# Orange-OpenSource/AIVC

Hardware: AMD Instinct MI355X
Metric: encode+decode fps @1080p YUV420 (RA GOP32) (higher is better)
Workload: dtype f32; 1 GPU; 1920x1080 8-bit YUV420, coding structure 1_GOP_32: one 128-frame clip = 4 intra-period units of 33 frames (132 coded frames, the last 4 repeat the last frame) encoded + decoded per step; synthetic random-init stand-in for model ms_ssim-4 (widths {'n2': 64, 'n': 128, 'c_y': 64, 'c_short': 64, 'c_z': 32, 'n_h': 128}), last analysis conv calibrated so that 6 (MOFNet) / 12 (CodecNet) of the 64 y featu; parallelism=single GPU

## Files before the change

aivc_amd/csrc/common.h:

```cpp
#pragma once
#include <hip/hip_runtime.h>
#include <stdint.h>

#include <atomic>

#include "../../include/aivc_detmath.h"
#include "../../include/aivc_hip.h"

#define AIVC_EXPORT extern "C" __attribute__((visibility("default")))

namespace aivc {

void set_last_error(const char *msg);
int check_launch(const char *what);

struct LdsOptIn {
  std::atomic<uint64_t> done{0};
  bool raise(const void *fn, size_t bytes) {
    int dev = 0;
    if (hipGetDevice(&dev) != hipSuccess) return false;
    const uint64_t bit = 1ull << (dev & 63);
    if (done.load(std::memory_order_acquire) & bit) return true;
    if (hipFuncSetAttribute(fn, hipFuncAttributeMaxDynamicSharedMemorySize, (int)bytes) != hipSuccess) return false;
    done.fetch_or(bit, std::memory_order_release);
    return true;
  }
};

constexpr uint64_t LOADER_MAX_BYTES = 0xFFFFFFF0ull;
static inline bool loader_addressable(uint64_t bytes) { return bytes <= LOADER_MAX_BYTES; }

static inline hipStream_t to_stream(aivc_stream_t s) { return reinterpret_cast<hipStream_t>(s); }
static inline unsigned cdiv(size_t a, size_t b) { return (unsigned)((a + b - 1) / b); }

__device__ __forceinline__ float act_apply(int act, float v) {
  switch (act) {
    case AIVC_ACT_LEAKY: return v > 0.0f ? v : v * 0.01f;
    case AIVC_ACT_RELU: return v > 0.0f ? v : 0.0f;
    case AIVC_ACT_SIGMOID: return aivc_sigmoidf_det(v);
    default: return v;
  }
}

constexpr float GDN_SAFE_LO = 0x1p-60f, GDN_SAFE_HI = 0x1p60f;
__device__ __forceinline__ float sqrt_rn_safe(float s) {
  const float y = __builtin_amdgcn_rsqf(s);
  float g = s * y, h = 0.5f * y;
  const float e = __builtin_fmaf(-h, g, 0.5f);
  h = __builtin_fmaf(h, e, h);
  g = __builtin_fmaf(g, e, g);
  const float d = __builtin_fmaf(-g, g, s);
  return __builtin_fmaf(d, h, g);
}
__device__ __forceinline__ float div_rn_safe(float v, float d) {
  float r = __builtin_amdgcn_rcpf(d);
  const float e = __builtin_fmaf(-d, r, 1.0f);
  r = __builtin_fmaf(e, r, r);
  float q = v * r;
  float t = __builtin_fmaf(-d, q, v);
  q = __builtin_fmaf(t, r, q);
  t = __builtin_fmaf(-d, q, v);
  return __builtin_fmaf(t, r, q);
}
__device__ __forceinline__ void gdn_range(float &mx, float &mn, float a, float s) {
  mx = __builtin_fmaxf(__builtin_fmaxf(mx, __builtin_fabsf(a)), s);
  mn = __builtin_fminf(__builtin_fminf(mn, __builtin_fabsf(a)), s);
}
__device__ __forceinline__ void gdn_range_pair(float &mx, float &mn, float s0, float s1) {
  mx = __builtin_fmaxf(__builtin_fmaxf(mx, s0), s1);
  mn = __builtin_fminf(__builtin_fminf(mn, s0), s1);
}
__device__ __forceinline__ bool gdn_range_ok(float mx, float mn) {
  return __builtin_amdgcn_ballot_w64(mn >= GDN_SAFE_LO && mx <= GDN_SAFE_HI) == __builtin_amdgcn_ballot_w64(true);
}

struct Epilogue {
  const float *bias, *mul, *res, *xin;
  float *y;
  int act1, act2, mode;
  __device__ __forceinline__ void store(size_t opix, int co, int c_out, float acc) const {
    float v = acc;
    if (bias) v = v + bias[co];
    if (mode == AIVC_MODE_GDN || mode == AIVC_MODE_IGDN) {
      const float xc = xin[opix * c_out + co];
      const float nrm = __builtin_sqrtf(v);
      v = (mode == AIVC_MODE_IGDN) ? xc * nrm : xc / nrm;
    }
    finish(opix, co, c_out, v);
  }
  __device__ __forceinline__ void finish(size_t opix, int co, int c_out, float v) const {
    v = act_apply(act1, v);
    const size_t o = opix * c_out + co;
    if (mul) v = mul[o] * v;
    if (res) v = v + res[o];
    v = act_apply(act2, v);
    y[o] = v;
  }
};

int conv2d_direct(const aivc_conv_params &p, hipStream_t s);
int conv2d_mfma(const aivc_conv_params &p, hipStream_t s);
bool conv2d_mfma_addressable(const aivc_conv_params &p);
bool conv2d_mfma_supported(const aivc_conv_params &p);
bool conv2d_mfma_tail_supported(const aivc_conv_params &p);
int conv2d_mfma_variant(const aivc_conv_params &p);
bool conv2d_bf16x3_supported(const aivc_conv_params &p);
int conv2d_bf16x3(const aivc_conv_params &p, hipStream_t s);
int split_weights_bf16x3(const float *w, int c_out, int k_total, void *out, hipStream_t s);
int conv2d_bf16x3_tile(const aivc_conv_params &p);
bool conv2d_wino_supported(const aivc_conv_params &p);
int conv2d_wino(const aivc_conv_params &p, hipStream_t s);
int conv2d_wino_variant(const aivc_conv_params &p);
int winograd_weights(const float *w, int c_out, int c_in, float *u, hipStream_t s);
int winograd_weights_poly5(const float *w, int c_out, int c_in, float *u, hipStream_t s);
int winograd_weights_tconv5(const float *w, int c_out, int c_in, float *u, hipStream_t s);
bool gdn_resident_supported(const aivc_conv_params &p);
int gdn_resident(const aivc_conv_params &p, hipStream_t s);
bool conv_images_supported(const aivc_image_src *src, int n_img, const aivc_conv_params &p);
int conv_images(const aivc_image_src *src, int n_img, const aivc_conv_params &p, hipStream_t s);
bool conv2d_thin_supported(const aivc_conv_params &p);
int conv2d_thin(const aivc_conv_params &p, hipStream_t s);
int conv2d_thin_variant(const aivc_conv_params &p);

}
```

aivc_amd/csrc/gdn.hip:

```cpp
#include <stdlib.h>

#include "mfma_util.h"

namespace aivc {

struct GdnArgs {
  aivc_conv_params p;
  int M;
  int ntiles;
};

constexpr int GDN_BM = 64;

__device__ __forceinline__ int gdn_swz(int row) { return (row & 15) ^ ((row & 4) << 1); }

template <int C>
struct GdnCfg {
  static constexpr int NB = C / 32;
  static constexpr int PW = C == 64 ? 2 : 1;
  static constexpr int NW = NB * PW;
  static constexpr int TM = 2 / PW;
  static constexpr int ROWB = C * 4;
  static constexpr int STAGE = GDN_BM * ROWB;
  static constexpr int PIECES = STAGE / 1024;
  static constexpr int PPW = (PIECES + NW - 1) / NW;
  static constexpr int WGS = C == 192 ? 1 : 2;
};

template <int C, bool INV, bool RES>
__global__ __launch_bounds__(64 * GdnCfg<C>::NW, GdnCfg<C>::WGS) void gdn_resident_kernel(GdnArgs a) {
  using Cfg = GdnCfg<C>;
  constexpr int NB = Cfg::NB, PW = Cfg::PW, NW = Cfg::NW, TM = Cfg::TM, ROWB = Cfg::ROWB, STAGE = Cfg::STAGE, PIECES = Cfg::PIECES, PPW = Cfg::PPW;
  constexpr int NOCT = C / 8;
  extern __shared__ __attribute__((aligned(16))) char gsmem[];
  const uint32_t lds0 = (uint32_t)(uintptr_t)(__attribute__((address_space(3))) char *)gsmem;
  const aivc_conv_params &p = a.p;
  const int tid = threadIdx.x, lane = tid & 63;
  const int wave = __builtin_amdgcn_readfirstlane(tid >> 6);
  const int nb = wave % NB, pw = wave / NB;
  const int l31 = lane & 31, hh = lane >> 5;
  const int M = a.M;

  float4 gb[NOCT];
  {
    const float *g = p.w + (size_t)(32 * nb + l31) * C + 4 * hh;
#pragma unroll
    for (int o = 0; o < NOCT; ++o) gb[o] = *reinterpret_cast<const float4 *>(g + 8 * o);
  }
  const float cbeta = p.bias[32 * nb + l31];

  uint32_t d_voff[PPW];
#pragma unroll
  for (int k = 0; k < PPW; ++k) {
    const int q = wave + NW * k;
    const int b = q * 1024 + lane * 16;
    const int row = b / ROWB, chunk = ((b % ROWB) >> 4) ^ gdn_swz(row);
    d_voff[k] = (uint32_t)(row * ROWB + chunk * 16);
  }
  const uint32_t w_dst = __builtin_amdgcn_readfirstlane(lds0 + (uint32_t)wave * 1024u);
  auto issue = [&](int tile, int stage) {
    const int m0 = tile * GDN_BM;
    const float *src = p.x + (size_t)m0 * C;
    const uint32_t dst = w_dst + (uint32_t)(stage * STAGE);
    if (m0 + GDN_BM <= M) {
#pragma unroll
      for (int k = 0; k < PPW; ++k)
        if (PIECES % NW == 0 || wave + NW * k < PIECES) glds16(src, d_voff[k], dst + (uint32_t)(NW * k) * 1024u);
    } else {
      const int last = M - 1 - m0;
#pragma unroll
      for (int k = 0; k < PPW; ++k)
        if (PIECES % NW == 0 || wave + NW * k < PIECES)
          glds16(src, (uint32_t)min((int)(d_voff[k] / ROWB), last) * (uint32_t)ROWB + d_voff[k] % ROWB, dst + (uint32_t)(NW * k) * 1024u);
    }
  };

  const int frow = (PW == 2 ? 32 * pw : 0) + l31;
  int f_off[8];
#pragma unroll
  for (int o = 0; o < 8; ++o) f_off[o] = frow * ROWB + (((2 * o + hh) ^ gdn_swz(frow)) << 4);
  const int e_chunk = (8 * nb + (l31 >> 2)) ^ (hh ? 12 : 0);
  const int e_lane = 4 * hh * ROWB + (l31 & 3) * 4;
  const int rb0 = PW == 2 ? 32 * pw : 0;

  const int G = gridDim.x;
  int tile = blockIdx.x;
  if (tile >= a.ntiles) return;
  issue(tile, 0);
  int stage = 0;
  for (; tile < a.ntiles; tile += G, stage ^= 1) {
    asm volatile("s_waitcnt vmcnt(0)" ::: "memory");
    __builtin_amdgcn_s_barrier();
    if (tile + G < a.ntiles) issue(tile + G, stage ^ 1);
    const char *sb = gsmem + stage * STAGE;

    floatx16 acc[TM];
    typedef float f32x2 __attribute__((ext_vector_type(2)));
    struct Frag { f32x2 lo, hi; };
    Frag cur[TM], nxt[TM];
    auto read_frag = [&](Frag (&f)[TM], int o) {
#pragma unroll
      for (int i = 0; i < TM; ++i) {
        const float4 v = *reinterpret_cast<const float4 *>(sb + f_off[o & 7] + (o >> 3) * 256 + i * 32 * ROWB);
        f[i].lo = (f32x2){v.x, v.y};
        f[i].hi = (f32x2){v.z, v.w};
      }
    };
    read_frag(cur, 0);
#pragma unroll
    for (int o = 0; o < NOCT; ++o) {
      if (o + 1 < NOCT) read_frag(nxt, o + 1);
#pragma unroll
      for (int i = 0; i < TM; ++i) {
        cur[i].lo = cur[i].lo * cur[i].lo;
        cur[i].hi = cur[i].hi * cur[i].hi;
      }
      __builtin_amdgcn_sched_barrier(0);
#pragma unroll
      for (int s = 0; s < 4; ++s) {
        const float bv = s == 0 ? gb[o].x : (s == 1 ? gb[o].y : (s == 2 ? gb[o].z : gb[o].w));
#pragma unroll
        for (int i = 0; i < TM; ++i) {
          const float av = s == 0 ? cur[i].lo.x : (s == 1 ? cur[i].lo.y : (s == 2 ? cur[i].hi.x : cur[i].hi.y));
          if (o == 0 && s == 0) {
            const floatx16 zero = {0.0f, 0.0f, 0.0f, 0.0f, 0.0f, 0.0f, 0.0f, 0.0f, 0.0f, 0.0f, 0.0f, 0.0f, 0.0f, 0.0f, 0.0f, 0.0f};
            acc[i] = __builtin_amdgcn_mfma_f32_32x32x2f32(av, bv, zero, 0, 0, 0);
          } else {
            acc[i] = __builtin_amdgcn_mfma_f32_32x32x2f32(av, bv, acc[i], 0, 0, 0);
          }
        }
      }
      __builtin_amdgcn_sched_barrier(0);
#pragma unroll
      for (int i = 0; i < TM; ++i) cur[i] = nxt[i];
    }

    const int m0 = tile * GDN_BM;
    const int rows_left = M - m0;
    typedef __attribute__((address_space(1))) char gchar;
    typedef __attribute__((address_space(1))) float gfloat;
    typedef __attribute__((address_space(1))) const float cgfloat;
    gchar *yb = (gchar *)(uintptr_t)(p.y + (size_t)m0 * C);
    const gchar *rsb = (const gchar *)(uintptr_t)(p.res + (size_t)m0 * C);
    const uint32_t lane_b = (uint32_t)((4 * hh) * ROWB + (32 * nb + l31) * 4);
    auto epilogue = [&](auto WHOLE) {
      constexpr bool whole = decltype(WHOLE)::value;
      constexpr int EG = RES ? 4 : 8;
#pragma unroll
      for (int i = 0; i < TM; ++i)
#pragma unroll
      for (int r0 = 0; r0 < 16; r0 += EG) {
        const int rb = rb0 + 32 * i;
        float xv[EG], sv[EG], rv[EG];
        float mx = 1.0f, mn = 1.0f;
#pragma unroll
        for (int q = 0; q < EG; ++q) {
          const int r = r0 + q, rloc = (r & 3) + 8 * (r >> 2);
          const int cst = (r & 3) | (((r >> 2) & 1) << 3);
          xv[q] = *reinterpret_cast<const float *>(sb + (rb + rloc) * ROWB + e_lane + ((e_chunk ^ cst) << 4));
          if constexpr (RES) {
            const uint32_t off = lane_b + (uint32_t)((rb + rloc) * ROWB);
            rv[q] = (whole || rb + rloc + 4 * hh < rows_left) ? *reinterpret_cast<cgfloat *>(rsb + off) : 0.0f;
          }
        }
#pragma unroll
        for (int q = 0; q < EG; ++q) {
          sv[q] = acc[i][r0 + q] + cbeta;
          if constexpr (INV) gdn_range_pair(mx, mn, sv[q], sv[q]);
          else gdn_range(mx, mn, xv[q], sv[q]);
        }
        if (gdn_range_ok(mx, mn)) {
#pragma unroll
          for (int q = 0; q < EG; ++q) {
            const float nrm = sqrt_rn_safe(sv[q]);
            float v = INV ? xv[q] * nrm : div_rn_safe(xv[q], nrm);
            if constexpr (RES) v = v + rv[q];
            sv[q] = v;
          }
        } else {
#pragma unroll
          for (int q = 0; q < EG; ++q) {
            const float nrm = __builtin_sqrtf(sv[q]);
            float v = INV ? xv[q] * nrm : xv[q] / nrm;
            if constexpr (RES) v = v + rv[q];
            sv[q] = v;
            if (q & 1) __builtin_amdgcn_sched_barrier(0);
          }
        }
#pragma unroll
        for (int q = 0; q < EG; ++q) {
          const int r = r0 + q, rloc = (r & 3) + 8 * (r >> 2);
          const uint32_t off = lane_b + (uint32_t)((rb + rloc) * ROWB);
          if (whole || rb + rloc + 4 * hh < rows_left) *reinterpret_cast<gfloat *>(yb + off) = sv[q];
        }
        __builtin_amdgcn_sched_barrier(0);
      }
    };
    if (rows_left >= GDN_BM) epilogue(std::true_type{});
    else epilogue(std::false_type{});
  }
}

bool gdn_resident_supported(const aivc_conv_params &p) {
  if (p.mode != AIVC_MODE_GDN && p.mode != AIVC_MODE_IGDN) return false;
  if (p.c_in != 64 && p.c_in != 128) return false;
  if (p.c_out != p.c_in || !p.bias || p.mul || p.act1 != AIVC_ACT_NONE || p.act2 != AIVC_ACT_NONE) return false;
  if (((uintptr_t)p.x & 15u) || ((uintptr_t)p.w & 15u)) return false;
  const uint64_t pix = (uint64_t)p.n * p.h_in * p.w_in;
  return pix >= 1 && pix < 0x7FFFFFC0ull;
}

template <int C, bool INV, bool RES>
static int gdn_launch(const GdnArgs &a, hipStream_t s, int n_cu) {
  using Cfg = GdnCfg<C>;
  constexpr size_t lds = 2 * (size_t)Cfg::STAGE;
  static LdsOptIn opt_in;
  if (!opt_in.raise(reinterpret_cast<const void *>(gdn_resident_kernel<C, INV, RES>), lds)) return check_launch("gdn_resident lds attribute");
  unsigned grid = (unsigned)(n_cu * Cfg::WGS);
  if ((unsigned)a.ntiles < grid) grid = (unsigned)a.ntiles;
  hipLaunchKernelGGL((gdn_resident_kernel<C, INV, RES>), dim3(grid), dim3(64 * Cfg::NW), lds, s, a);
  return check_launch("gdn_resident");
}

int gdn_resident(const aivc_conv_params &p, hipStream_t s) {
  if (!gdn_resident_supported(p)) return AIVC_ERR_UNSUPPORTED;
  GdnArgs a;
  a.p = p;
  a.M = p.n * p.h_in * p.w_in;
  a.ntiles = (a.M + GDN_BM - 1) / GDN_BM;
  static std::atomic<int> n_cu{0};
  if (n_cu.load(std::memory_order_relaxed) == 0) {
    int dev = 0, cus = 0;
    n_cu = hipGetDevice(&dev) == hipSuccess && hipDeviceGetAttribute(&cus, hipDeviceAttributeMultiprocessorCount, dev) == hipSuccess && cus > 0 ? cus : 256;
  }
  const int cus = n_cu.load(std::memory_order_relaxed);
  const bool inv = p.mode == AIVC_MODE_IGDN, res = p.res != nullptr;
  auto go = [&](auto CC) {
    constexpr int C = decltype(CC)::value;
    if (inv) return res ? gdn_launch<C, true, true>(a, s, cus) : gdn_launch<C, true, false>(a, s, cus);
    return res ? gdn_launch<C, false, true>(a, s, cus) : gdn_launch<C, false, false>(a, s, cus);
  };
  if (p.c_in == 64) return go(std::integral_constant<int, 64>{});
  return go(std::integral_constant<int, 128>{});
}

}
```

aivc_amd/csrc/selfcheck.hip:

```cpp
#include "common.h"

namespace aivc {

__global__ __launch_bounds__(256) void selfcheck_sqrt_kernel(uint32_t first, uint32_t last, unsigned long long *bad) {
  unsigned long long n = 0;
  for (uint64_t b = (uint64_t)first + (uint64_t)blockIdx.x * 256 + threadIdx.x; b <= last; b += (uint64_t)gridDim.x * 256) {
    const float s = __uint_as_float((uint32_t)b);
    n += __float_as_uint(sqrt_rn_safe(s)) != __float_as_uint(__builtin_sqrtf(s));
  }
  if (n) atomicAdd(bad, n);
}

__device__ __forceinline__ uint64_t mix64(uint64_t z) {
  z = (z ^ (z >> 30)) * 0xBF58476D1CE4E5B9ull;
  z = (z ^ (z >> 27)) * 0x94D049BB133111EBull;
  return z ^ (z >> 31);
}

__global__ __launch_bounds__(256) void selfcheck_div_kernel(uint64_t n_pairs, uint32_t seed, unsigned long long *bad) {
  unsigned long long n = 0;
  for (uint64_t i = (uint64_t)blockIdx.x * 256 + threadIdx.x; i < n_pairs; i += (uint64_t)gridDim.x * 256) {
    const uint64_t h = mix64(i + ((uint64_t)seed << 32) + 0x9E3779B97F4A7C15ull), h2 = mix64(h);
    const uint32_t ev = 127u - 60u + (uint32_t)((h >> 23) % 120u), ed = 127u - 30u + (uint32_t)((h2 >> 23) % 60u);
    uint32_t mv = (uint32_t)h & 0x7FFFFFu;
    const uint32_t md = (uint32_t)h2 & 0x7FFFFFu;
    if ((i & 3) == 3) mv = (md + (uint32_t)((h >> 50) & 7u) - 3u) & 0x7FFFFFu;
    const float v = __uint_as_float(((uint32_t)(h >> 63) << 31) | (ev << 23) | mv);
    const float d = __uint_as_float((ed << 23) | md);
    n += __float_as_uint(div_rn_safe(v, d)) != __float_as_uint(v / d);
  }
  if (n) atomicAdd(bad, n);
}

}

AIVC_EXPORT int aivc_selfcheck_gdn_math(uint64_t n_div_pairs, uint32_t seed, uint64_t *mismatch, aivc_stream_t stream) {
  if (!mismatch) return AIVC_ERR_ARG;
  hipStream_t s = aivc::to_stream(stream);
  if (hipMemsetAsync(mismatch, 0, 2 * sizeof(uint64_t), s) != hipSuccess) return aivc::check_launch("selfcheck memset");
  const uint32_t first = __builtin_bit_cast(uint32_t, aivc::GDN_SAFE_LO), last = __builtin_bit_cast(uint32_t, aivc::GDN_SAFE_HI);
  hipLaunchKernelGGL(aivc::selfcheck_sqrt_kernel, dim3(4096), dim3(256), 0, s, first, last, reinterpret_cast<unsigned long long *>(mismatch));
  if (n_div_pairs)
    hipLaunchKernelGGL(aivc::selfcheck_div_kernel, dim3(4096), dim3(256), 0, s, n_div_pairs, seed, reinterpret_cast<unsigned long long *>(mismatch) + 1);
  return aivc::check_launch("selfcheck_gdn_math");
}

namespace aivc {

template <typename T>
__global__ __launch_bounds__(256) void detmath_eval_kernel(int fn, const T *__restrict__ a, const T *__restrict__ b, size_t n, T *__restrict__ out) {
  for (size_t i = (size_t)blockIdx.x * 256 + threadIdx.x; i < n; i += (size_t)gridDim.x * 256) {
    if constexpr (sizeof(T) == 8) {
      const double x = a[i];
      double r;
      switch (fn) {
        case AIVC_DETMATH_EXP: r = aivc_det_exp(x); break;
        case AIVC_DETMATH_EXPM1: r = aivc_det_expm1(x); break;
        case AIVC_DETMATH_LOG: r = aivc_det_log(x); break;
        default: r = aivc_det_log1p(x); break;
      }
      out[i] = r;
    } else {
      const float x = a[i];
      float r;
      switch (fn) {
        case AIVC_DETMATH_EXPF: r = aivc_expf_det(x); break;
        case AIVC_DETMATH_EXPM1F: r = aivc_expm1f_det(x); break;
        case AIVC_DETMATH_SIGMOIDF: r = aivc_sigmoidf_det(x); break;
        case AIVC_DETMATH_TANHF: r = aivc_tanhf_det(x); break;
        case AIVC_DETMATH_SOFTPLUSF: r = aivc_softplusf_det(x); break;
        case AIVC_DETMATH_POWF: r = aivc_powf_det(x, b[i]); break;
        default: r = aivc_laplace_cdf(x, b[i]); break;
      }
      out[i] = r;
    }
  }
}

}

AIVC_EXPORT int aivc_detmath_eval(int32_t fn, const void *a, const void *b, size_t n, void *out, aivc_stream_t stream) {
  if (fn < 0 || fn >= AIVC_DETMATH_COUNT) return AIVC_ERR_ARG;
  if (n == 0) return AIVC_OK;
  const bool two = fn == AIVC_DETMATH_POWF || fn == AIVC_DETMATH_LAPLACE_CDF;
  if (!a || !out || (two && !b)) return AIVC_ERR_ARG;
  hipStream_t s = aivc::to_stream(stream);
  const unsigned blocks = aivc::cdiv(n, 256) < 8192u ? aivc::cdiv(n, 256) : 8192u;
  if (fn <= AIVC_DETMATH_LOG1P)
    hipLaunchKernelGGL(aivc::detmath_eval_kernel<double>, dim3(blocks), dim3(256), 0, s, (int)fn, static_cast<const double *>(a),
                       static_cast<const double *>(b), n, static_cast<double *>(out));
  else
    hipLaunchKernelGGL(aivc::detmath_eval_kernel<float>, dim3(blocks), dim3(256), 0, s, (int)fn, static_cast<const float *>(a),
                       static_cast<const float *>(b), n, static_cast<float *>(out));
  return aivc::check_launch("detmath_eval");
}
```

Baseline: 102.1 frames/s.

## Transpose GDN MFMA output for residual variant to enable float4 epilogue

For the residual GDN kernel, the MFMA operands are swapped so each lane holds four consecutive channels of one pixel. The epilogue can then read x, the residual and the bias as float4 vectors and write y with float4 stores. Residual loads are hoisted before the MMA loop to overlap their latency, and packed 2-wide sqrt/div helpers are added to use paired FP32 math. Supported cases now also require 16-byte alignment of y, res and bias, and the selfcheck tests the packed math helpers.

After: 102.5 frames/s, median of 6. No clear change (+0.3%).

```diff
diff --git a/aivc_amd/csrc/common.h b/aivc_amd/csrc/common.h
--- a/aivc_amd/csrc/common.h
+++ b/aivc_amd/csrc/common.h
@@ -62,6 +62,28 @@
   t = __builtin_fmaf(-d, q, v);
   return __builtin_fmaf(t, r, q);
 }
+typedef float f32x2 __attribute__((ext_vector_type(2)));
+__device__ __forceinline__ f32x2 sqrt_rn_safe2(f32x2 s) {
+  const f32x2 y = {__builtin_amdgcn_rsqf(s.x), __builtin_amdgcn_rsqf(s.y)};
+  const f32x2 half = {0.5f, 0.5f};
+  f32x2 g = s * y, h = half * y;
+  const f32x2 e = __builtin_elementwise_fma(-h, g, half);
+  h = __builtin_elementwise_fma(h, e, h);
+  g = __builtin_elementwise_fma(g, e, g);
+  const f32x2 d = __builtin_elementwise_fma(-g, g, s);
+  return __builtin_elementwise_fma(d, h, g);
+}
+__device__ __forceinline__ f32x2 div_rn_safe2(f32x2 v, f32x2 d) {
+  f32x2 r = {__builtin_amdgcn_rcpf(d.x), __builtin_amdgcn_rcpf(d.y)};
+  const f32x2 one = {1.0f, 1.0f};
+  const f32x2 e = __builtin_elementwise_fma(-d, r, one);
+  r = __builtin_elementwise_fma(e, r, r);
+  f32x2 q = v * r;
+  f32x2 t = __builtin_elementwise_fma(-d, q, v);
+  q = __builtin_elementwise_fma(t, r, q);
+  t = __builtin_elementwise_fma(-d, q, v);
+  return __builtin_elementwise_fma(t, r, q);
+}
 __device__ __forceinline__ void gdn_range(float &mx, float &mn, float a, float s) {
   mx = __builtin_fmaxf(__builtin_fmaxf(mx, __builtin_fabsf(a)), s);
   mn = __builtin_fminf(__builtin_fminf(mn, __builtin_fabsf(a)), s);
diff --git a/aivc_amd/csrc/gdn.hip b/aivc_amd/csrc/gdn.hip
--- a/aivc_amd/csrc/gdn.hip
+++ b/aivc_amd/csrc/gdn.hip
@@ -32,6 +32,7 @@
   using Cfg = GdnCfg<C>;
   constexpr int NB = Cfg::NB, PW = Cfg::PW, NW = Cfg::NW, TM = Cfg::TM, ROWB = Cfg::ROWB, STAGE = Cfg::STAGE, PIECES = Cfg::PIECES, PPW = Cfg::PPW;
   constexpr int NOCT = C / 8;
+  constexpr bool QUADS = RES;
   extern __shared__ __attribute__((aligned(16))) char gsmem[];
   const uint32_t lds0 = (uint32_t)(uintptr_t)(__attribute__((address_space(3))) char *)gsmem;
   const aivc_conv_params &p = a.p;
@@ -47,7 +48,14 @@
 #pragma unroll
     for (int o = 0; o < NOCT; ++o) gb[o] = *reinterpret_cast<const float4 *>(g + 8 * o);
   }
-  const float cbeta = p.bias[32 * nb + l31];
+  float cbeta = 0.0f;
+  float4 qbeta[4];
+  if constexpr (QUADS) {
+#pragma unroll
+    for (int g = 0; g < 4; ++g) qbeta[g] = *reinterpret_cast<const float4 *>(p.bias + 32 * nb + 8 * g + 4 * hh);
+  } else {
+    cbeta = p.bias[32 * nb + l31];
+  }
 
   uint32_t d_voff[PPW];
 #pragma unroll
@@ -79,9 +87,18 @@
   int f_off[8];
 #pragma unroll
   for (int o = 0; o < 8; ++o) f_off[o] = frow * ROWB + (((2 * o + hh) ^ gdn_swz(frow)) << 4);
+  const int rb0 = PW == 2 ? 32 * pw : 0;
   const int e_chunk = (8 * nb + (l31 >> 2)) ^ (hh ? 12 : 0);
   const int e_lane = 4 * hh * ROWB + (l31 & 3) * 4;
-  const int rb0 = PW == 2 ? 32 * pw : 0;
+  const uint32_t lane_b = (uint32_t)((4 * hh) * ROWB + (32 * nb + l31) * 4);
+  const int q_off = frow * ROWB + (((8 * nb + hh) ^ gdn_swz(frow)) << 4);
+  const uint32_t q_lane_b = (uint32_t)(frow * ROWB + (32 * nb + 4 * hh) * 4);
+
+  typedef float gfloat4 __attribute__((ext_vector_type(4)));
+  typedef __attribute__((address_space(1))) char gchar;
+  typedef __attribute__((address_space(1))) float gfloat;
+  typedef __attribute__((address_space(1))) gfloat4 ggfloat4;
+  typedef __attribute__((address_space(1))) const gfloat4 cggfloat4;
 
   const int G = gridDim.x;
   int tile = blockIdx.x;
@@ -93,9 +110,23 @@
     __builtin_amdgcn_s_barrier();
     if (tile + G < a.ntiles) issue(tile + G, stage ^ 1);
     const char *sb = gsmem + stage * STAGE;
+    const int m0 = tile * GDN_BM;
+    const int rows_left = M - m0;
+    gchar *yb = (gchar *)(uintptr_t)(p.y + (size_t)m0 * C);
+    gfloat4 rres[RES ? TM : 1][4];
+    if constexpr (RES) {
+      const gchar *rsb = (const gchar *)(uintptr_t)(p.res + (size_t)m0 * C);
+#pragma unroll
+      for (int i = 0; i < TM; ++i)
+#pragma unroll
+        for (int g = 0; g < 4; ++g) {
+          rres[i][g] = (gfloat4){0.0f, 0.0f, 0.0f, 0.0f};
+          if (rows_left >= GDN_BM || rb0 + 32 * i + l31 < rows_left)
+            rres[i][g] = *reinterpret_cast<cggfloat4 *>(rsb + (q_lane_b + (uint32_t)(i * 32 * ROWB + g * 32)));
+        }
+    }
 
     floatx16 acc[TM];
-    typedef float f32x2 __attribute__((ext_vector_type(2)));
     struct Frag { f32x2 lo, hi; };
     Frag cur[TM], nxt[TM];
     auto read_frag = [&](Frag (&f)[TM], int o) {
@@ -118,16 +149,13 @@
       __builtin_amdgcn_sched_barrier(0);
 #pragma unroll
       for (int s = 0; s < 4; ++s) {
-        const float bv = s == 0 ? gb[o].x : (s == 1 ? gb[o].y : (s == 2 ? gb[o].z : gb[o].w));
+        const float gv = s == 0 ? gb[o].x : (s == 1 ? gb[o].y : (s == 2 ? gb[o].z : gb[o].w));
 #pragma unroll
         for (int i = 0; i < TM; ++i) {
-          const float av = s == 0 ? cur[i].lo.x : (s == 1 ? cur[i].lo.y : (s == 2 ? cur[i].hi.x : cur[i].hi.y));
-          if (o == 0 && s == 0) {
-            const floatx16 zero = {0.0f, 0.0f, 0.0f, 0.0f, 0.0f, 0.0f, 0.0f, 0.0f, 0.0f, 0.0f, 0.0f, 0.0f, 0.0f, 0.0f, 0.0f, 0.0f};
-            acc[i] = __builtin_amdgcn_mfma_f32_32x32x2f32(av, bv, zero, 0, 0, 0);
-          } else {
-            acc[i] = __builtin_amdgcn_mfma_f32_32x32x2f32(av, bv, acc[i], 0, 0, 0);
-          }
+          const float sq = s == 0 ? cur[i].lo.x : (s == 1 ? cur[i].lo.y : (s == 2 ? cur[i].hi.x : cur[i].hi.y));
+          const floatx16 zero = {0.0f, 0.0f, 0.0f, 0.0f, 0.0f, 0.0f, 0.0f, 0.0f, 0.0f, 0.0f, 0.0f, 0.0f, 0.0f, 0.0f, 0.0f, 0.0f};
+          const floatx16 from = o == 0 && s == 0 ? zero : acc[i];
+          acc[i] = QUADS ? __builtin_amdgcn_mfma_f32_32x32x2f32(gv, sq, from, 0, 0, 0) : __builtin_amdgcn_mfma_f32_32x32x2f32(sq, gv, from, 0, 0, 0);
         }
       }
       __builtin_amdgcn_sched_barrier(0);
@@ -135,33 +163,21 @@
       for (int i = 0; i < TM; ++i) cur[i] = nxt[i];
     }
 
-    const int m0 = tile * GDN_BM;
-    const int rows_left = M - m0;
-    typedef __attribute__((address_space(1))) char gchar;
-    typedef __attribute__((address_space(1))) float gfloat;
-    typedef __attribute__((address_space(1))) const float cgfloat;
-    gchar *yb = (gchar *)(uintptr_t)(p.y + (size_t)m0 * C);
-    const gchar *rsb = (const gchar *)(uintptr_t)(p.res + (size_t)m0 * C);
-    const uint32_t lane_b = (uint32_t)((4 * hh) * ROWB + (32 * nb + l31) * 4);
-    auto epilogue = [&](auto WHOLE) {
+    auto epilogue_rows = [&](auto WHOLE) {
       constexpr bool whole = decltype(WHOLE)::value;
-      constexpr int EG = RES ? 4 : 8;
+      constexpr int EG = 8;
 #pragma unroll
       for (int i = 0; i < TM; ++i)
 #pragma unroll
       for (int r0 = 0; r0 < 16; r0 += EG) {
         const int rb = rb0 + 32 * i;
-        float xv[EG], sv[EG], rv[EG];
+        float xv[EG], sv[EG];
         float mx = 1.0f, mn = 1.0f;
 #pragma unroll
         for (int q = 0; q < EG; ++q) {
           const int r = r0 + q, rloc = (r & 3) + 8 * (r >> 2);
           const int cst = (r & 3) | (((r >> 2) & 1) << 3);
           xv[q] = *reinterpret_cast<const float *>(sb + (rb + rloc) * ROWB + e_lane + ((e_chunk ^ cst) << 4));
-          if constexpr (RES) {
-            const uint32_t off = lane_b + (uint32_t)((rb + rloc) * ROWB);
-            rv[q] = (whole || rb + rloc + 4 * hh < rows_left) ? *reinterpret_cast<cgfloat *>(rsb + off) : 0.0f;
-          }
         }
 #pragma unroll
         for (int q = 0; q < EG; ++q) {
@@ -173,17 +189,13 @@
 #pragma unroll
           for (int q = 0; q < EG; ++q) {
             const float nrm = sqrt_rn_safe(sv[q]);
-            float v = INV ? xv[q] * nrm : div_rn_safe(xv[q], nrm);
-            if constexpr (RES) v = v + rv[q];
-            sv[q] = v;
+            sv[q] = INV ? xv[q] * nrm : div_rn_safe(xv[q], nrm);
           }
         } else {
 #pragma unroll
           for (int q = 0; q < EG; ++q) {
             const float nrm = __builtin_sqrtf(sv[q]);
-            float v = INV ? xv[q] * nrm : xv[q] / nrm;
-            if constexpr (RES) v = v + rv[q];
-            sv[q] = v;
+            sv[q] = INV ? xv[q] * nrm : xv[q] / nrm;
             if (q & 1) __builtin_amdgcn_sched_barrier(0);
           }
         }
@@ -195,6 +207,74 @@
         }
         __builtin_amdgcn_sched_barrier(0);
       }
+    };
+    auto epilogue_quads = [&](auto WHOLE) {
+      constexpr bool whole = decltype(WHOLE)::value;
+      constexpr int EQ = 1;
+#pragma unroll
+      for (int i = 0; i < TM; ++i) {
+        const bool live = whole || rb0 + 32 * i + l31 < rows_left;
+#pragma unroll
+        for (int g0 = 0; g0 < 4; g0 += EQ) {
+          gfloat4 xv[EQ], rv[EQ];
+          f32x2 sv[EQ][2];
+          float mx = 1.0f, mn = 1.0f;
+#pragma unroll
+          for (int q = 0; q < EQ; ++q) {
+            const int g = g0 + q;
+            xv[q] = *reinterpret_cast<const gfloat4 *>(sb + (q_off ^ (g << 5)) + i * 32 * ROWB);
+            if constexpr (RES) rv[q] = rres[i][g];
+            sv[q][0] = (f32x2){acc[i][4 * g], acc[i][4 * g + 1]} + (f32x2){qbeta[g].x, qbeta[g].y};
+            sv[q][1] = (f32x2){acc[i][4 * g + 2], acc[i][4 * g + 3]} + (f32x2){qbeta[g].z, qbeta[g].w};
+          }
+#pragma unroll
+          for (int q = 0; q < EQ; ++q) {
+            if constexpr (INV) {
+              gdn_range_pair(mx, mn, sv[q][0].x, sv[q][0].y);
+              gdn_range_pair(mx, mn, sv[q][1].x, sv[q][1].y);
+            } else {
+              gdn_range(mx, mn, xv[q].x, sv[q][0].x);
+              gdn_range(mx, mn, xv[q].y, sv[q][0].y);
+              gdn_range(mx, mn, xv[q].z, sv[q][1].x);
+              gdn_range(mx, mn, xv[q].w, sv[q][1].y);
+            }
+          }
+          if (gdn_range_ok(mx, mn)) {
+#pragma unroll
+            for (int q = 0; q < EQ; ++q)
+#pragma unroll
+              for (int h = 0; h < 2; ++h) {
+                const f32x2 x2 = h ? (f32x2){xv[q].z, xv[q].w} : (f32x2){xv[q].x, xv[q].y};
+                const f32x2 nrm = sqrt_rn_safe2(sv[q][h]);
+                f32x2 v = INV ? x2 * nrm : div_rn_safe2(x2, nrm);
+                if constexpr (RES) v = v + (h ? (f32x2){rv[q].z, rv[q].w} : (f32x2){rv[q].x, rv[q].y});
+                sv[q][h] = v;
+              }
+          } else {
+#pragma unroll
+            for (int q = 0; q < EQ; ++q)
+#pragma unroll
+              for (int e = 0; e < 4; ++e) {
+                const float nrm = __builtin_sqrtf(sv[q][e >> 1][e & 1]);
+                float v = INV ? xv[q][e] * nrm : xv[q][e] / nrm;
+                if constexpr (RES) v = v + rv[q][e];
+                sv[q][e >> 1][e & 1] = v;
+                if (e & 1) __builtin_amdgcn_sched_barrier(0);
+              }
+          }
+          if (live) {
+#pragma unroll
+            for (int q = 0; q < EQ; ++q)
+              *reinterpret_cast<ggfloat4 *>(yb + (q_lane_b + (uint32_t)(i * 32 * ROWB + (g0 + q) * 32))) =
+                  (gfloat4){sv[q][0].x, sv[q][0].y, sv[q][1].x, sv[q][1].y};
+          }
+          __builtin_amdgcn_sched_barrier(0);
+        }
+      }
+    };
+    auto epilogue = [&](auto WHOLE) {
+      if constexpr (QUADS) epilogue_quads(WHOLE);
+      else epilogue_rows(WHOLE);
     };
     if (rows_left >= GDN_BM) epilogue(std::true_type{});
     else epilogue(std::false_type{});
@@ -206,6 +286,7 @@
   if (p.c_in != 64 && p.c_in != 128) return false;
   if (p.c_out != p.c_in || !p.bias || p.mul || p.act1 != AIVC_ACT_NONE || p.act2 != AIVC_ACT_NONE) return false;
   if (((uintptr_t)p.x & 15u) || ((uintptr_t)p.w & 15u)) return false;
+  if (p.res && ((((uintptr_t)p.y | (uintptr_t)p.res | (uintptr_t)p.bias)) & 15u)) return false;
   const uint64_t pix = (uint64_t)p.n * p.h_in * p.w_in;
   return pix >= 1 && pix < 0x7FFFFFC0ull;
 }
diff --git a/aivc_amd/csrc/selfcheck.hip b/aivc_amd/csrc/selfcheck.hip
--- a/aivc_amd/csrc/selfcheck.hip
+++ b/aivc_amd/csrc/selfcheck.hip
@@ -6,7 +6,11 @@
   unsigned long long n = 0;
   for (uint64_t b = (uint64_t)first + (uint64_t)blockIdx.x * 256 + threadIdx.x; b <= last; b += (uint64_t)gridDim.x * 256) {
     const float s = __uint_as_float((uint32_t)b);
-    n += __float_as_uint(sqrt_rn_safe(s)) != __float_as_uint(__builtin_sqrtf(s));
+    const float t = __uint_as_float(first + (last - (uint32_t)b));
+    const uint32_t ws = __float_as_uint(__builtin_sqrtf(s)), wt = __float_as_uint(__builtin_sqrtf(t));
+    const f32x2 st = sqrt_rn_safe2((f32x2){s, t}), ts = sqrt_rn_safe2((f32x2){t, s});
+    n += __float_as_uint(sqrt_rn_safe(s)) != ws;
+    n += __float_as_uint(st.x) != ws || __float_as_uint(st.y) != wt || __float_as_uint(ts.x) != wt || __float_as_uint(ts.y) != ws;
   }
   if (n) atomicAdd(bad, n);
 }
@@ -27,7 +31,11 @@
     if ((i & 3) == 3) mv = (md + (uint32_t)((h >> 50) & 7u) - 3u) & 0x7FFFFFu;
     const float v = __uint_as_float(((uint32_t)(h >> 63) << 31) | (ev << 23) | mv);
     const float d = __uint_as_float((ed << 23) | md);
-    n += __float_as_uint(div_rn_safe(v, d)) != __float_as_uint(v / d);
+    const float d2 = __uint_as_float(__float_as_uint(d) ^ 0x2AAAAAu);
+    const uint32_t w = __float_as_uint(v / d), w2 = __float_as_uint(d / d2);
+    const f32x2 a = div_rn_safe2((f32x2){v, d}, (f32x2){d, d2}), b = div_rn_safe2((f32x2){d, v}, (f32x2){d2, d});
+    n += __float_as_uint(div_rn_safe(v, d)) != w;
+    n += __float_as_uint(a.x) != w || __float_as_uint(a.y) != w2 || __float_as_uint(b.x) != w2 || __float_as_uint(b.y) != w;
   }
   if (n) atomicAdd(bad, n);
 }
```
